# TravisWheelerLab/BATH

Hardware: AMD Instinct MI355X
Metric: DP Gcells/s + residues/s through bathsearch pipeline at 1/2/4/8 MI355X (higher is better)
Workload: dtype u8/i16 integer scores (SSV: exact binary16), f32 Forward

## Files before the change

bath_amd/__init__.py:

```python
import ctypes as C
import os
import subprocess

import numpy as np

_HERE = os.path.dirname(os.path.abspath(__file__))
_ROOT = os.path.dirname(_HERE)
LIB_PATH = os.environ.get("BATH_HIP_LIBRARY") or os.path.join(_HERE, "libbathhip.so")

OK, EINVAL, ERANGE, ENORESULT = 0, 11, 16, 19
KP, K, NEVPARAM = 29, 20, 8
LOGSUM_TABLE, LOGSUM_EXACT, LOGSUM_TABLE_SERIAL, LOGSUM_CONTEXT = 0, 1, 2, 3
LOGSUM_ODDS = 4
ENSEMBLE_SERIAL, ENSEMBLE_STREAMS_HOST, ENSEMBLE_STREAMS_DEVICE = 0, 1, 2
ENSEMBLE_MODES = {"serial": ENSEMBLE_SERIAL, "streams": ENSEMBLE_STREAMS_HOST, "device": ENSEMBLE_STREAMS_DEVICE}
ENS_SAMPLES = 200
ARITH_STRICT, ARITH_ODDS3, ARITH_ODDS = 0, 1, 2
ARITH_MODES = {"strict": ARITH_STRICT, "odds3": ARITH_ODDS3, "odds": ARITH_ODDS}
ENS_OK, ENS_IMPOSSIBLE, ENS_STEP_CAP, ENS_SEG_OVERFLOW = 0, 1, 2, 3
ENS_REGION_OK, ENS_REGION_NO_TRACES = 0, 1

DNA_SYMS = "ACGT-RYMKSWHBVDN*~"
AMINO_SYMS = "ACDEFGHIKLMNPQRSTVWY-BJZOUX*~"

# ... 150 lines not shown
    "bath_hmmfile_count": (C.c_int, [C.c_char_p]),
    "bath_hmmfile_read": (C.c_int, [C.c_char_p, C.c_int, C.POINTER(C.POINTER(_Hmm))]),
    "bath_hmm_destroy": (None, [C.POINTER(_Hmm)]),
    "bath_gencode_basic": (C.c_int, [C.c_int, _u8p]),
    "bath_profile_config": (C.c_int, [C.POINTER(_Hmm), C.c_int, C.POINTER(C.POINTER(_Profile))]),
    "bath_profile_destroy": (None, [C.POINTER(_Profile)]),
    "bath_fs_profile_config": (C.c_int, [C.POINTER(_Hmm), _u8p, C.c_int, C.c_int, C.POINTER(C.POINTER(_FsProfile))]),
    "bath_fs_profile_destroy": (None, [C.POINTER(_FsProfile)]),
    "bath_hip_init": (C.c_int, [C.c_int, C.POINTER(_vp)]),
    "bath_hip_finalize": (None, [_vp]),
    "bath_hip_last_error": (C.c_char_p, [_vp]),
    "bath_hip_synchronize": (C.c_int, [_vp]),
    "bath_hip_stream": (_vp, [_vp]),
    "bath_hip_set_fs_strict": (C.c_int, [_vp, C.c_int]),
    "bath_hip_set_fwd_group": (C.c_int, [_vp, C.c_int]),
    "bath_hip_set_fs_serial": (C.c_int, [_vp, C.c_int]),
    "bath_hip_set_fs_odds": (C.c_int, [_vp, C.c_int]),
    "bath_hip_set_fs5_odds": (C.c_int, [_vp, C.c_int]),
    "bath_hip_set_fs_ensemble": (C.c_int, [_vp, C.c_int]),
    "bath_hip_fs_ensemble_counters": (C.c_int, [_vp, _i64p, _i64p, _i64p]),
    "bath_hip_set_std_ensemble": (C.c_int, [_vp, C.c_int]),
    "bath_hip_std_ensemble_counters": (C.c_int, [_vp, _i64p, _i64p, _i64p]),
    "bath_hip_std_region_ensembles": (C.c_int, [_vp, _vp, _vp, _i32p, C.c_uint32, _i32p, _i32p, _i32p, C.c_int64, _i64p, _i32p, _f32p, C.c_int64, _i64p]),
    "bath_selftest_std_ensemble": (C.c_int, [C.c_int, C.c_int, _f32p, _f32p, C.c_float, C.c_float, C.c_float, _u8p, C.c_int, _f32p, _f32p, C.c_uint32, _i32p, _i32p,
                                             _i32p, C.c_int, _i32p, _f32p, _i32p, C.c_int, _i32p]),
    "bath_selftest_std_ens_walk": (C.c_int, [C.c_int, _f32p, C.c_float, C.c_float, C.c_float, C.c_int, _f32p, _f32p, C.c_uint32, _i32p, _i32p, C.c_int, _i32p]),
    "bath_hip_fs5_region_ensembles": (C.c_int, [_vp, _vp, _vp, C.c_uint32, _i32p, _i32p, _i32p, C.c_int64, _i64p, _i32p, C.c_int64, _i64p]),
    "bath_selftest_fs_ensemble_seeded": (C.c_int, [C.c_int, _f32p, C.c_float, C.c_float, C.c_float, C.c_int, C.c_int, _f32p, _f32p, C.c_uint32, _i32p, C.c_int, _i32p]),
    "bath_selftest_fs_ensemble_streams": (C.c_int, [C.c_int, _f32p, C.c_float, C.c_float, C.c_float, C.c_int, C.c_int, _f32p, _f32p, C.c_uint32,
                                                    _i32p, _i32p, _i32p, C.c_int, _i32p, _i32p, C.c_int, _i32p]),
# ... 297 lines not shown
        if st != OK:
            raise BathError("%s failed (%d): %s" % (what, st, lib().bath_hip_last_error(self._h).decode()))

    def synchronize(self):
        self._check(lib().bath_hip_synchronize(self._h), "synchronize")

    def trim(self):
        self._check(lib().bath_hip_trim(self._h), "trim")

    def set_fs_strict(self, on=True):
        self._check(lib().bath_hip_set_fs_strict(self._h, 1 if on else 0), "set_fs_strict")

    def set_fwd_group(self, mode):
        self._check(lib().bath_hip_set_fwd_group(self._h, int(mode)), "set_fwd_group")

    def set_fs_odds(self, on=True):
        self._check(lib().bath_hip_set_fs_odds(self._h, 1 if on else 0), "set_fs_odds")

    def set_fs5_odds(self, on=True):
        self._check(lib().bath_hip_set_fs5_odds(self._h, 1 if on else 0), "set_fs5_odds")

    def set_fs_ensemble(self, mode):
        self._check(lib().bath_hip_set_fs_ensemble(self._h, ENSEMBLE_MODES.get(mode, mode)), "set_fs_ensemble")

    def fs_ensemble_counters(self):
        a, b, c = C.c_int64(0), C.c_int64(0), C.c_int64(0)
        self._check(lib().bath_hip_fs_ensemble_counters(self._h, C.byref(a), C.byref(b), C.byref(c)), "fs_ensemble_counters")
        return {"bound_fallbacks": a.value, "overflow_fallbacks": b.value, "matrix_bytes_kept": c.value}

    def set_std_ensemble(self, mode):
# ... 1279 lines not shown
```

bath_amd/csrc/bath_common.hpp:

```cpp
#pragma once
#include <set>
#include <atomic>
#include <hip/hip_runtime.h>

#include <cstdint>
#include <chrono>
#include <cstdio>
#include <cstdlib>
#include <cstring>
#include <condition_variable>
#include <functional>
#include <mutex>
#include <string>
#include <thread>
#include <vector>

#include "bath_hip.h"
#include "bath_tilings.hpp"
#include "bath_slots.hpp"

namespace bath {

inline hipError_t allow_max_lds(const void *fn) {
  static std::mutex mu;
// ... 116 lines not shown

}

struct bath_hip_ctx;
namespace bath {
extern std::atomic<int> g_ctx_total, g_ctx_internal;
inline int host_contexts() { return g_ctx_total.load() - g_ctx_internal.load(); }
inline void mark_internal(bath_hip_ctx *c);
}
struct bath_hip_ctx {
  int device = 0;
  hipStream_t stream = nullptr;
  hipStream_t tail_stream = nullptr;
  hipStream_t side_stream = nullptr;
  hipEvent_t ev_fork = nullptr, ev_join = nullptr;
  hipStream_t copy_stream = nullptr;
  hipDeviceProp_t prop{};
  int fs_strict = 1;
  int fs_odds = 0;
  int fs5_odds = 0;
  int fwd_group = 0;
  int fs_ensemble = 0;
  std::atomic<int64_t> fs_ens_bound_fallbacks{0}, fs_ens_overflow_fallbacks{0}, fs_ens_bytes_kept{0};
  int std_ensemble = 0;
  std::atomic<int64_t> std_ens_serial_fallbacks{0}, std_ens_twin_fallbacks{0}, std_ens_kernel_regions{0};
  int fs_serial = -1;
  uint64_t tabs_uid = 0;
  const void *tabs_ptr = nullptr;
  uint64_t fsw_pad_uid = 0;
  int orf_tables_id = -1;
  std::string err;
  void set_error(const std::string &m) { err = m; }
  std::vector<float> fsw_len_terms;
  bath::SlotArray<bath::Scratch, bath::DevBuf> scratch;
  bath::SlotArray<bath::Pinned, bath::HostBuf> stage;
  template <class T> int stage_upload(bath::Pinned slot, void *dst, const T *src, size_t n, hipStream_t s) {
// ... 187 lines not shown
```

bath_amd/csrc/bath_pipeline.hip:

```cpp
#include <algorithm>
#include <cmath>
#include <cstring>
#include <cstdlib>
#include <map>
#include <thread>

#include "bath_common.hpp"
#include "bath_kernels.hpp"
#include "bath_launch.hpp"
#include "host_model.hpp"

using namespace bath;

namespace bath {

static const double kLog2 = 0.69314718055994529;

enum { FLAG_VIT_RUN = 1, FLAG_HAS_WIN = 2 };

struct Counters {
  int cand_count, todo_msv, todo_vit, todo_ssvb, todo_vit2, todo_fwd, win_count, overflow;
  int todo_lb;
  int fwd_next;
  unsigned long long n_orfs, orf_res;
  unsigned long long n_past_msv, n_past_bias, n_past_vit, n_past_fwd;
  unsigned long long pos_past_msv, pos_past_bias, pos_past_vit, pos_past_fwd;
  unsigned long long res_vit, res_fwd;
  unsigned long long res_seen;
};

struct Params {
  double F1, F2, F3, F4;
  int do_bias, fs_pipe, minlen;
  float evparam[BATH_NEVPARAM];
};

template <int NR, int G>
// ... 378 lines not shown
  for (int dx = 0; dx < 6; dx++) {
    float n0 = 0.f, n1 = 0.f, den = 0.f;
    if (dx == 5) { for (int y = 0; y < 20; y++) { n0 += bgf[y]; n1 += compo[y]; den += bgf[y]; } }
    else {
      const int a = min(mem[dx][0], mem[dx][1]), b = max(mem[dx][0], mem[dx][1]);
      n0 += bgf[a]; n1 += compo[a]; den += bgf[a];
      if (b != a) { n0 += bgf[b]; n1 += compo[b]; den += bgf[b]; }
    }
    eo[2 * (21 + dx)] = den > 0.f ? n0 / den : 0.f;
    eo[2 * (21 + dx) + 1] = den > 0.f ? n1 / den : 0.f;
  }
}

enum { PV_TODO_LB = 0, PV_TODO_FWD = 1, PV_NL = 2 };
enum { PV_N_VIT = 0, PV_POS_VIT, PV_RES_FWD, PV_NS };
__global__ __launch_bounds__(256) void post_vit_kernel(Cand cand, int cand_cap, Counters *__restrict__ ctr, Params p, int32_t *__restrict__ todo_lb, int32_t *__restrict__ todo_fwd) {
  __shared__ BlockTally<PV_NL, PV_NS, 512> tally;
  tally_reset(tally);
  const TallyOut<PV_NL, PV_NS> out{{todo_lb, todo_fwd}, {&ctr->todo_lb, &ctr->todo_fwd}, {&ctr->n_past_vit, &ctr->pos_past_vit, &ctr->res_fwd}};
  const int ncand = min(ctr->cand_count, cand_cap);
  for (int c0 = blockIdx.x * blockDim.x; c0 < ncand; c0 += gridDim.x * blockDim.x) {
    if (tally_lists_full(tally)) tally_write_lists(tally, out);
    const int c = c0 + threadIdx.x;
    bool past = c < ncand && cand.stage[c] == 2;
    if (past && (cand.flags[c] & FLAG_VIT_RUN)) {
      const float seqsc = (float)((double)(cand.vfsc[c] - cand.filtersc[c]) / kLog2);
      const double P = d_gumbel_surv(seqsc, p.evparam[2], p.evparam[3]);
      cand.P[c] = P;
      if (P > p.F2) { cand.kminmax[2 * c] = 1 << 30; cand.kminmax[2 * c + 1] = 0; past = false; }
    }
    if (!past) continue;
    const int L = cand.len[c];
    tally_add(tally, PV_N_VIT, 1ull); tally_add(tally, PV_POS_VIT, (unsigned long long)L * 3ull);
    if (p.do_bias && cand.kminmax[2 * c] <= cand.kminmax[2 * c + 1]) {
      cand.flags[c] |= FLAG_HAS_WIN;
      tally_push(tally, PV_TODO_LB, c);
      continue;
    }
    cand.stage[c] = 3;
    tally_push(tally, PV_TODO_FWD, c); tally_add(tally, PV_RES_FWD, (unsigned long long)L);
  }
  tally_finish(tally, out);
}

__host__ __device__ __forceinline__ float compo_term(float bg, int base_b, int sc, float scale_b) {
  const float lo = ((float)base_b - (float)sc) / scale_b;
  return bg * expf(lo);
}
__global__ void compo_terms_kernel(const float *__restrict__ bgf, int base_b, float scale_b, float *__restrict__ terms ) {
  const int x = blockIdx.x, sc = threadIdx.x;
  terms[x * 256 + sc] = compo_term(bgf[x], base_b, sc, scale_b);
}

__global__ __launch_bounds__(64) void local_compo_kernel(Cand cand, const Counters *__restrict__ ctr, int M, const uint8_t *__restrict__ ssv_scores,
                                                         const float *__restrict__ terms, const int32_t *__restrict__ todo_lb, float *__restrict__ compo_out ) {
  const int lane = threadIdx.x, g = lane / 20, x = lane % 20;
  const int ntodo = ctr->todo_lb;
  for (int base = blockIdx.x * 3; base < ntodo; base += gridDim.x * 3) {
    const int job = base + g;
    if (g >= 3 || job >= ntodo) continue;
    const int c = todo_lb[job];
    int k_start = cand.kminmax[2 * c], k_end = cand.kminmax[2 * c + 1];
    const int k_len = k_end - k_start + 1;
    if (k_len < 20) { k_start -= (20 - k_len) / 2; k_end += (20 - k_len) / 2; }
    k_start = max(1, k_start); k_end = min(M, k_end);
    const float *tx = terms + x * 256;
    float acc = 0.0f;
    for (int k = k_start; k <= k_end; k++) acc += tx[ssv_scores[(size_t)k * kKp + x]];
    compo_out[(size_t)job * 20 + x] = acc;
  }
}

__global__ __launch_bounds__(64) void post_vit_local_kernel(Cand cand, Counters *__restrict__ ctr, Params p, const uint8_t *__restrict__ pool, int M,
                                                            const float *__restrict__ bgf, const float *__restrict__ compo_in,
                                                            const float *__restrict__ p1_tab, const float *__restrict__ lt1_tab, const float *__restrict__ lt2_tab,
                                                            const int32_t *__restrict__ todo_lb, int32_t *__restrict__ todo_vit2, int32_t *__restrict__ todo_fwd) {
  __shared__ float s_eo[64][kKp * 2 + 1];
  __shared__ BlockTally<2, 2, 128> tally;
  tally_reset(tally);
  const TallyOut<2, 2> out{{todo_vit2, todo_fwd}, {&ctr->todo_vit2, &ctr->todo_fwd}, {&ctr->res_vit, &ctr->res_fwd}};
  const int ntodo = ctr->todo_lb;
  for (int job0 = blockIdx.x * blockDim.x; job0 < ntodo; job0 += gridDim.x * blockDim.x) {
    if (tally_lists_full(tally)) tally_write_lists(tally, out);
    const int job = job0 + threadIdx.x;
    if (job >= ntodo) continue;
    const int c = todo_lb[job];
    const int L = cand.len[c];
    const float usc = cand.usc[c];
    float filtersc = cand.filtersc[c];
    const float vfsc = (cand.flags[c] & FLAG_VIT_RUN) ? cand.vfsc[c] : -INFINITY;
    float compo[20];
    for (int y = 0; y < 20; y++) compo[y] = compo_in[(size_t)job * 20 + y];
    float *eo = s_eo[threadIdx.x];
    local_compo_finish(compo, bgf, eo);
    float lf = bias_forward(pool + cand.off[c], L, M, eo, p1_tab[L]);
    lf = (lf + lt1_tab[L]) + lt2_tab[L];
// ... 115 lines not shown
  float *d_bgf = om->d_compo_terms + 20 * 256;
  BATH_HIP_TRY(ctx, hipMemcpyAsync(d_bgf, kAminoBg, 20 * sizeof(float), hipMemcpyHostToDevice, ctx->stream));
  hipLaunchKernelGGL(compo_terms_kernel, dim3(20), dim3(256), 0, ctx->stream, d_bgf, (int)om->base_b, om->scale_b, om->d_compo_terms);
  BATH_HIP_TRY(ctx, hipGetLastError());
  BATH_HIP_TRY(ctx, hipStreamSynchronize(ctx->stream));
  return BATH_OK;
}

static int wave_grid_blocks(bath_hip_ctx *ctx) { return ctx->prop.multiProcessorCount * 8; }

struct PipelineWork {
  Cand cand;
  int cand_cap = 0;
  uint8_t *pool = nullptr;
  int32_t *todo_msv = nullptr, *todo_vit = nullptr, *todo_ssvb = nullptr, *todo_vit2 = nullptr, *todo_fwd = nullptr, *todo_sorted = nullptr;
  int *len_bins = nullptr;
  WindowRec *wins = nullptr;
  int win_cap = 0;
  Counters *ctr = nullptr;
};

template <class T>
static T *carve(char *&p, size_t n) {
  T *r = reinterpret_cast<T *>(p);
  p += (n * sizeof(T) + 255) / 256 * 256;
  return r;
}

static size_t layout(PipelineWork &w, char *base, int cap, int win_cap) {
  char *p = base;
// ... 1 lines not shown
  w.cand_cap = cap; w.win_cap = std::max(2 * cap, win_cap);
  if (win_cap == 0) {
    static const int forced = [] { const char *e = std::getenv("BATH_HIP_TEST_WINCAP"); return e ? std::atoi(e) : 0; }();
    if (forced > 0) w.win_cap = forced;
  }
  w.ctr = carve<Counters>(p, 1);
  w.cand.window = carve<int64_t>(p, n); w.cand.off = carve<int64_t>(p, n); w.cand.P = carve<double>(p, n);
  w.cand.sf = carve<int32_t>(p, n); w.cand.startj = carve<int32_t>(p, n); w.cand.len = carve<int32_t>(p, n);
  w.cand.msv_status = carve<int32_t>(p, n); w.cand.vit_status = carve<int32_t>(p, n); w.cand.fwd_status = carve<int32_t>(p, n); w.cand.stage = carve<int32_t>(p, n);
  w.cand.flags = carve<int32_t>(p, n); w.cand.kminmax = carve<int32_t>(p, 2 * n);
  w.cand.usc = carve<float>(p, n); w.cand.nullsc = carve<float>(p, n); w.cand.filtersc = carve<float>(p, n);
  w.cand.vfsc = carve<float>(p, n); w.cand.fwdsc = carve<float>(p, n);
  w.cand.v = carve<int16_t>(p, n);
  w.todo_msv = carve<int32_t>(p, n); w.todo_vit = carve<int32_t>(p, n); w.todo_ssvb = carve<int32_t>(p, n);
  w.todo_vit2 = carve<int32_t>(p, n); w.todo_fwd = carve<int32_t>(p, n); w.todo_sorted = carve<int32_t>(p, n);
  w.len_bins = carve<int>(p, 2048);
  w.wins = carve<WindowRec>(p, (size_t)w.win_cap);
  return (size_t)(p - base);
}

}

extern "C" int bath_selftest_compo_terms(int base_b, float scale_b, float *terms) {
  if (!terms || !(scale_b > 0.f)) return BATH_EINVAL;
  for (int x = 0; x < 20; x++)
    for (int sc = 0; sc < 256; sc++) terms[x * 256 + sc] = bath::compo_term(kAminoBg[x], base_b, sc, scale_b);
  return BATH_OK;
}

extern "C" void bath_pipeline_params_default(bath_pipeline_params *p, int fs_pipe) {
// ... 190 lines not shown
      BATH_HIP_TRY(ctx, hipEventRecord(ev[e++], ctx->stream));
    } else {
      hipLaunchKernelGGL(classify_kernel, dim3(dec_blocks), dim3(256), 0, ctx->stream, W.cand, W.cand_cap, W.ctr, om->lt.d_tjb, mc, W.todo_msv);
      BATH_HIP_TRY(ctx, hipGetLastError());
      if ((st = launch_msv_wave(ctx, om, cv, W.todo_msv, cap, W.cand.usc, W.cand.msv_status, &W.ctr->todo_msv, !few_msv)) != BATH_OK) return st;
      BATH_HIP_TRY(ctx, hipEventRecord(ev[e++], ctx->stream));
      hipLaunchKernelGGL(f1_bias_kernel, dim3(dec_blocks), dim3(256), 0, ctx->stream, W.cand, W.cand_cap, W.ctr, P, W.pool, M, f1t, W.todo_vit, W.todo_ssvb);
      BATH_HIP_TRY(ctx, hipGetLastError());
      BATH_HIP_TRY(ctx, hipEventRecord(ev[e++], ctx->stream));
    }
    wa.d_filtersc = W.cand.filtersc; wa.d_ssv_scores = d_ssvsc; wa.d_wins = W.wins; wa.d_win_count = &W.ctr->win_count; wa.win_cap = W.win_cap;
    wa.d_kminmax = W.cand.kminmax;
    auto launch_ssvb = [&](hipStream_t stream) -> int {
      return launch_ssv_bath(ctx, stream, om, W.cand, W.ctr, W.todo_ssvb, W.pool, d_ssvsc, mc, invP_f1, W.wins, W.win_cap);
    };
    bool ssvb_done = false;
    if (vit_lane_supported(om) && !few_cands) {
      if ((st = launch_vit_sorted(ctx, om, cv, W.todo_vit, cap, &W.ctr->todo_vit, W.cand.len, W.len_bins, W.todo_sorted, W.cand.vfsc, W.cand.vit_status, &wa,
                                  launch_ssvb)) != BATH_OK) return st;
      ssvb_done = true;
    } else if ((st = launch_vit_wave(ctx, om, cv, W.todo_vit, cap, W.cand.vfsc, W.cand.vit_status, &wa, &W.ctr->todo_vit)) != BATH_OK) return st;
    BATH_HIP_TRY(ctx, hipEventRecord(ev[e++], ctx->stream));
    if (!ssvb_done && (st = launch_ssvb(ctx->stream)) != BATH_OK) return st;
    BATH_HIP_TRY(ctx, hipGetLastError());
    BATH_HIP_TRY(ctx, hipEventRecord(ev[e++], ctx->stream));
    hipLaunchKernelGGL(post_vit_kernel, dim3(dec_blocks), dim3(256), 0, ctx->stream, W.cand, W.cand_cap, W.ctr, P, W.todo_msv , W.todo_fwd);
    if (P.do_bias) {
      DevBuf &b_compo = ctx->scratch[Scratch::kLocalCompoSums];
      BATH_HIP_TRY(ctx, b_compo.reserve((size_t)W.cand_cap * 20 * 4 + 256));
      float *d_compo = b_compo.as<float>();
      hipLaunchKernelGGL(local_compo_kernel, dim3(16384), dim3(64), 0, ctx->stream, W.cand, W.ctr, M, d_ssvsc, om->d_compo_terms, W.todo_msv, d_compo);
      hipLaunchKernelGGL(post_vit_local_kernel, dim3(std::max(1, dec_blocks)), dim3(64), 0, ctx->stream, W.cand, W.ctr, P, W.pool, M, d_bgf, d_compo,
                         om->lt.d_p1, om->lt.d_lt1, om->lt.d_lt2, W.todo_msv, W.todo_vit2, W.todo_fwd);
    }
    BATH_HIP_TRY(ctx, hipGetLastError());
    if ((st = launch_vit_wave(ctx, om, cv, W.todo_vit2, cap, W.cand.vfsc, W.cand.vit_status, nullptr, &W.ctr->todo_vit2)) != BATH_OK) return st;
    hipLaunchKernelGGL(post_vit2_kernel, dim3(64), dim3(256), 0, ctx->stream, W.cand, W.ctr, P, W.todo_vit2, W.todo_fwd);
    BATH_HIP_TRY(ctx, hipGetLastError());
    BATH_HIP_TRY(ctx, hipEventRecord(ev[e++], ctx->stream));
    ctx->fwd_rows_kept = nullptr; ctx->fwd_rows_off = nullptr;
    float *d_keep = nullptr; int64_t *d_keep_off = nullptr;
    if (ctx->keep_fwd_rows) {
      constexpr int64_t kKeepFloats = (int64_t)8 << 20;
      DevBuf &b_rows = ctx->scratch[Scratch::kCascadeFwdRows], &b_roff = ctx->scratch[Scratch::kCascadeFwdRowOffsets];
      BATH_HIP_TRY(ctx, b_rows.reserve((size_t)kKeepFloats * sizeof(float) + 64)); BATH_HIP_TRY(ctx, b_roff.reserve((size_t)cap * sizeof(int64_t) + 64));
      d_keep = b_rows.as<float>(); d_keep_off = b_roff.as<int64_t>();
      hipLaunchKernelGGL(fwd_keep_offsets_kernel, dim3(1), dim3(64), 0, ctx->stream, W.todo_fwd, &W.ctr->todo_fwd, W.cand.len, d_keep_off, kKeepFloats);
      BATH_HIP_TRY(ctx, hipGetLastError());
    }
    const bool fwd_group = !d_keep && fwd_group_supported(om) && ctx->fwd_group != 2;
    if (fwd_group) {
      if ((st = launch_len_sort(ctx, W.todo_fwd, &W.ctr->todo_fwd, W.cand.len, W.len_bins, W.todo_sorted)) != BATH_OK) return st;
// ... 2 lines not shown
    const int64_t fwd_launches = (d_keep ? 1 : 0) + (fwd_group ? 4 : 1) + 1;
    if (d_keep) { ctx->fwd_rows_kept = d_keep; ctx->fwd_rows_off = d_keep_off; }
    hipLaunchKernelGGL(final_kernel, dim3(dec_blocks), dim3(256), 0, ctx->stream, W.cand, W.ctr, P, W.todo_fwd);
    BATH_HIP_TRY(ctx, hipGetLastError());
    BATH_HIP_TRY(ctx, hipEventRecord(ev[e++], ctx->stream));

    BATH_HIP_TRY(ctx, hipMemcpyAsync(&hc, W.ctr, sizeof(Counters), hipMemcpyDeviceToHost, ctx->stream));
    BATH_HIP_TRY(ctx, hipStreamSynchronize(ctx->stream));
    if (hc.overflow || hc.cand_count > cap || hc.win_count > W.win_cap) {
      if (attempt >= 4) { ctx->set_error("candidate / window buffers overflowed repeatedly"); return BATH_EMEM; }
      if (hc.overflow || hc.cand_count > cap) cap = std::max<int64_t>(cap * 2, (int64_t)hc.cand_count + 1024);
      if (hc.win_count > W.win_cap) win_need = hc.win_count + hc.win_count / 4 + 1024;
      continue;
    }
    static const char *names[] = {"translate_orfs", "ssv_f1", "classify_msv", "f1_bias", "viterbi_windows", "ssv_windows", "post_vit", "forward_final"};
    const int64_t launches[] = {4, 1, msv_stage ? 1 : 2, msv_stage ? 0 : 1, 4, 1, 3, fwd_launches};
    ctx->timings.clear();
    for (int i = 0; i + 1 < e; i++) {
      float ms = 0.f;
      BATH_HIP_TRY(ctx, hipEventElapsedTime(&ms, ev[i], ev[i + 1]));
      ctx->timings.push_back(StageTiming{names[i], ms, launches[i]});
    }
    break;
  }

  if (stats) {
    stats->nres = nres; stats->n_orfs = (int64_t)hc.n_orfs;
    stats->n_past_msv = (int64_t)hc.n_past_msv; stats->n_past_bias = (int64_t)hc.n_past_bias;
    stats->n_past_vit = (int64_t)hc.n_past_vit; stats->n_past_fwd = (int64_t)hc.n_past_fwd;
    stats->pos_past_msv = (int64_t)hc.pos_past_msv; stats->pos_past_bias = (int64_t)hc.pos_past_bias;
    stats->pos_past_vit = (int64_t)hc.pos_past_vit; stats->pos_past_fwd = (int64_t)hc.pos_past_fwd;
// ... 87 lines not shown
    mark_internal(lane);
    const char *pe = std::getenv("BATH_HIP_LANE_PRIO");
    if (!(pe && pe[0] == '0')) {
      int lo = 0, hi = 0;
      if (hipDeviceGetStreamPriorityRange(&lo, &hi) == hipSuccess && lo != hi) {
        (void)hipStreamDestroy(lane->stream);
        const char *te = std::getenv("BATH_HIP_TAIL_PRIO");
        const bool tails = te && te[0] == '1';
        const int prio = tails ? (ctx->lanes.empty() ? std::min(lo, hi + 1) : lo) : (ctx->lanes.empty() ? hi : lo);
        if (hipStreamCreateWithPriority(&lane->stream, hipStreamNonBlocking, prio) != hipSuccess) { ctx->set_error("hipStreamCreateWithPriority"); return BATH_EFAIL; }
        if (tails && hipStreamCreateWithPriority(&lane->tail_stream, hipStreamNonBlocking, hi) != hipSuccess) { ctx->set_error("hipStreamCreateWithPriority"); return BATH_EFAIL; }
      }
    }
    ctx->lanes.push_back(lane);
  }
  for (bath_hip_ctx *lane : ctx->lanes) { lane->fs_strict = ctx->fs_strict; lane->fs_odds = ctx->fs_odds; lane->fs5_odds = ctx->fs5_odds; lane->fwd_group = ctx->fwd_group; }
  if ((st = ensure_parts(ctx, dna, K)) != BATH_OK) return st;
  std::vector<bath_pipeline_stats> pst((size_t)K);
  std::vector<const bath_orf_result *> pres((size_t)K, nullptr);
  std::vector<int64_t> pn((size_t)K, 0);
  std::vector<int> rc((size_t)K, BATH_OK);
  states->assign((size_t)K, FilterState{});
  if (!ctx->ev_lanes) BATH_HIP_TRY(ctx, hipEventCreateWithFlags(&ctx->ev_lanes, hipEventDisableTiming));
  BATH_HIP_TRY(ctx, hipEventRecord(ctx->ev_lanes, ctx->stream));
  for (int k = 0; k < K; k++) BATH_HIP_TRY(ctx, hipStreamWaitEvent(ctx->lanes[(size_t)k]->stream, ctx->ev_lanes, 0));
  if (!ctx->lane_pool) ctx->lane_pool = new LanePool();
  ctx->lane_pool->run(K, [&](int k) {
    bath_hip_ctx *lane = ctx->lanes[(size_t)k];
    rc[(size_t)k] = run_filters(lane, om, dna->parts[(size_t)k], prm, &pst[(size_t)k], results ? &pres[(size_t)k] : nullptr, &pn[(size_t)k], &(*states)[(size_t)k]);
    if (rc[(size_t)k] == BATH_OK) rc[(size_t)k] = after(k, lane, dna->parts[(size_t)k], (*states)[(size_t)k]);
  });
// ... 511 lines not shown
```

bath_amd/csrc/bath_profile.hip:

```cpp
#include <atomic>
#include <cctype>
#include <cmath>
#include <cstring>

#include "bath_common.hpp"
#include "host_model.hpp"

using namespace bath;

namespace bath {

static const double kLog2 = 0.69314718055994529;

double gumbel_surv(double x, double mu, double lambda) {
  double ey = -std::exp(-lambda * (x - mu));
  if (std::fabs(ey) < 5e-9) return -ey;
  return 1.0 - std::exp(ey);
}
double gumbel_invsurv(double p, double mu, double lambda) {
  double lp = (p < 5e-9) ? (std::pow(p, p) - 1) / p : std::log(-1. * std::log(1 - p));
  return mu - lp / lambda;
}
double exp_surv(double x, double mu, double lambda) { return (x < mu) ? 1.0 : std::exp(-lambda * (x - mu)); }

// ... 67 lines not shown

}

int bath_hip_oprofile::ensure_len_tables(int maxL) const { return bath::build_len_tables(this, maxL); }


namespace bath { std::atomic<int> g_ctx_total{0}, g_ctx_internal{0}; }

extern "C" int bath_hip_init(int device, bath_hip_ctx **out) {
  *out = nullptr;
  int ndev = 0;
  if (hipGetDeviceCount(&ndev) != hipSuccess || ndev <= 0) return BATH_ENODEVICE;
  if (device < 0 || device >= ndev) return BATH_EINVAL;
  bath_hip_ctx *ctx = new bath_hip_ctx();
  ctx->device = device;
  if (const char *e = std::getenv("BATH_HIP_SYNC")) {
    static const bool once = [&] {
      (void)hipSetDevice(device);
      const unsigned fl = (e[0] == 'b') ? hipDeviceScheduleBlockingSync : (e[0] == 'y') ? hipDeviceScheduleYield : hipDeviceScheduleSpin;
      if (hipSetDeviceFlags(fl) != hipSuccess) (void)hipGetLastError();
      return true;
    }();
    (void)once;
  }
  if (hipSetDevice(device) != hipSuccess || hipGetDeviceProperties(&ctx->prop, device) != hipSuccess ||
      hipStreamCreateWithFlags(&ctx->stream, hipStreamNonBlocking) != hipSuccess) {
    delete ctx;
    return BATH_ENODEVICE;
  }
  bath::g_ctx_total.fetch_add(1);
// ... 13 lines not shown
  if (ctx->ev_lanes) (void)hipEventDestroy(ctx->ev_lanes);
  if (ctx->tail_stream) (void)hipStreamDestroy(ctx->tail_stream);
  if (ctx->aux) { bath_hip_finalize(ctx->aux); ctx->aux = nullptr; }
  if (ctx->aux2) { bath_hip_finalize(ctx->aux2); ctx->aux2 = nullptr; }
  if (ctx->aux3) { bath_hip_finalize(ctx->aux3); ctx->aux3 = nullptr; }
  for (auto &b : ctx->scratch) b.release();
  for (auto &b : ctx->pinned) b.release();
  for (auto &b : ctx->stage) b.release();
  ctx->results_pinned.release();
  for (auto e : ctx->ev_pool) (void)hipEventDestroy(e);
  for (auto e : ctx->span_events) (void)hipEventDestroy(e);
  if (ctx->ev_fork) (void)hipEventDestroy(ctx->ev_fork);
  if (ctx->ev_join) (void)hipEventDestroy(ctx->ev_join);
  if (ctx->copy_stream) (void)hipStreamDestroy(ctx->copy_stream);
  if (ctx->side_stream) (void)hipStreamDestroy(ctx->side_stream);
  (void)hipStreamDestroy(ctx->stream);
  delete ctx;
}

extern "C" int bath_hip_trim(bath_hip_ctx *ctx) {
  if (!ctx) return BATH_EINVAL;
  BATH_HIP_TRY(ctx, hipSetDevice(ctx->device));
  BATH_HIP_TRY(ctx, hipStreamSynchronize(ctx->stream));
  delete ctx->lane_pool; ctx->lane_pool = nullptr;
  for (bath_hip_ctx *lane : ctx->lanes) bath_hip_finalize(lane);
  ctx->lanes.clear();
  if (ctx->aux) { bath_hip_finalize(ctx->aux); ctx->aux = nullptr; }
  if (ctx->aux2) { bath_hip_finalize(ctx->aux2); ctx->aux2 = nullptr; }
  if (ctx->aux3) { bath_hip_finalize(ctx->aux3); ctx->aux3 = nullptr; }
  if (ctx->tail_stream) { (void)hipStreamDestroy(ctx->tail_stream); ctx->tail_stream = nullptr; }
  if (ctx->copy_stream) { (void)hipStreamSynchronize(ctx->copy_stream); (void)hipStreamDestroy(ctx->copy_stream); ctx->copy_stream = nullptr; }
  if (ctx->side_stream) {
    (void)hipStreamSynchronize(ctx->side_stream); (void)hipStreamDestroy(ctx->side_stream); ctx->side_stream = nullptr;
    if (ctx->ev_fork) { (void)hipEventDestroy(ctx->ev_fork); ctx->ev_fork = nullptr; }
    if (ctx->ev_join) { (void)hipEventDestroy(ctx->ev_join); ctx->ev_join = nullptr; }
  }
  ctx->fs_std_orfs.clear(); ctx->fs_std_pool = nullptr; ctx->fs_keep_xoff.clear(); ctx->fs_regions_all.clear();
  ctx->d_records = nullptr; ctx->n_records = 0;
  return BATH_OK;
}

extern "C" const char *bath_hip_last_error(const bath_hip_ctx *ctx) { return ctx ? ctx->err.c_str() : "no context"; }

extern "C" int bath_hip_synchronize(bath_hip_ctx *ctx) {
  BATH_HIP_TRY(ctx, hipSetDevice(ctx->device));
  BATH_HIP_TRY(ctx, hipStreamSynchronize(ctx->stream));
  return BATH_OK;
}

extern "C" void *bath_hip_stream(bath_hip_ctx *ctx) { return (void *)ctx->stream; }
extern "C" int bath_hip_kernel_times(bath_hip_ctx *ctx, int max, bath_kernel_time *out) {
// ... 19 lines not shown
}

extern "C" int bath_hip_set_fs_strict(bath_hip_ctx *ctx, int on) {
  if (!ctx) return BATH_EINVAL;
  ctx->fs_strict = on ? 1 : 0;
  if (!on && ctx->aux3) { bath_hip_finalize(ctx->aux3); ctx->aux3 = nullptr; }
  for (bath_hip_ctx *l : ctx->lanes) l->fs_strict = ctx->fs_strict;
  return BATH_OK;
}

extern "C" int bath_hip_set_fwd_group(bath_hip_ctx *ctx, int mode) {
  if (!ctx) return BATH_EINVAL;
  if (mode < 0 || mode > 2) { ctx->set_error("bath_hip_set_fwd_group: mode must be 0, 1 or 2"); return BATH_EINVAL; }
  ctx->fwd_group = mode;
  for (bath_hip_ctx *l : ctx->lanes) l->fwd_group = mode;
  return BATH_OK;
}

extern "C" int bath_hip_set_fs_odds(bath_hip_ctx *ctx, int on) {
  if (!ctx) return BATH_EINVAL;
  ctx->fs_odds = on ? 1 : 0;
  for (bath_hip_ctx *l : ctx->lanes) l->fs_odds = ctx->fs_odds;
  return BATH_OK;
}

extern "C" int bath_hip_set_fs5_odds(bath_hip_ctx *ctx, int on) {
  if (!ctx) return BATH_EINVAL;
  ctx->fs5_odds = on ? 1 : 0;
  for (bath_hip_ctx *l : ctx->lanes) l->fs5_odds = ctx->fs5_odds;
  return BATH_OK;
// ... 471 lines not shown
```

bath_amd/csrc/bath_viterbi.hip:

```cpp
#include <algorithm>
#include <cstdlib>
#include <functional>

#include "bath_common.hpp"
#include "bath_kernels.hpp"
#include "bath_launch.hpp"

using namespace bath;

namespace bath {

__device__ __forceinline__ s16x2 pk_adds(s16x2 a, s16x2 b) { return __builtin_elementwise_add_sat(a, b); }
__device__ __forceinline__ s16x2 pk_max(s16x2 a, s16x2 b) { return __builtin_elementwise_max(a, b); }
__device__ __forceinline__ s16x2 as_s2(unsigned v) { return __builtin_bit_cast(s16x2, v); }
__device__ __forceinline__ unsigned as_u(s16x2 v) { return __builtin_bit_cast(unsigned, v); }

struct VitLaneTables {
  const int16_t *rw;
  int rw_pitch_bytes;
  const uint32_t *tw2;
  const int16_t *rank;
};

struct VitLaneConsts {
// ... 6 lines not shown

typedef uint32_t u32x16 __attribute__((ext_vector_type(16)));

template <int NR>
#ifndef BATH_VIT_WAVES
#define BATH_VIT_WAVES 1
#endif
__global__ __launch_bounds__(256, (NR <= 76 ? BATH_VIT_WAVES : 1)) void vit_lane_kernel(SeqView sq, VitLaneTables tb, const uint32_t *__restrict__ tw2g, VitLaneConsts c, const int16_t *__restrict__ xwmove_tab,
                                                          const uint8_t *__restrict__ tjb_tab, const int32_t *__restrict__ todo, int64_t ntodo,
                                                          const int *__restrict__ ntodo_dev, const int *__restrict__ skip_dev, float *__restrict__ sc, int32_t *__restrict__ status,
                                                          const float *__restrict__ filtersc, const uint8_t *__restrict__ ssv_scores,
                                                          WindowRec *__restrict__ wins, int *__restrict__ win_count, int win_cap, int32_t *__restrict__ kminmax) {
  extern __shared__ __attribute__((aligned(16))) char lds[];
  char *s_rw = lds;
  int16_t *s_rank = reinterpret_cast<int16_t *>(lds + 30 * tb.rw_pitch_bytes);
  {
    const uint32_t *src = reinterpret_cast<const uint32_t *>(tb.rw);
    uint32_t *dst = reinterpret_cast<uint32_t *>(s_rw);
    for (int i = threadIdx.x; i < 30 * tb.rw_pitch_bytes / 4; i += blockDim.x) dst[i] = src[i];
    for (int i = threadIdx.x; i < 2 * NR; i += blockDim.x) s_rank[i] = tb.rank[i];
  }
  __syncthreads();
  if (ntodo_dev) ntodo = *ntodo_dev;
  const int64_t t = (int64_t)blockIdx.x * blockDim.x + threadIdx.x + (skip_dev ? *skip_dev : 0);
  if (t - (threadIdx.x & 63) >= ntodo) return;
  const bool live = t < ntodo;
  const int64_t sid = live ? (todo ? (int64_t)todo[t] : t) : (todo ? (int64_t)todo[0] : 0);
  const int L = live ? sq.len[sid] : 0;
  const uint8_t *s = sq.data + sq.off[sid];
  const int Lw = wave_max_i32(L);
// ... 279 lines not shown
```

include/bath_hip.h:

```cpp
#ifndef BATH_HIP_H
#define BATH_HIP_H

#include <stdint.h>
#include <stddef.h>

#ifdef __cplusplus
extern "C" {
#endif

#define BATH_OK          0
#define BATH_EFAIL       1
#define BATH_EMEM        5
#define BATH_EFORMAT     7
#define BATH_EINVAL     11
#define BATH_ERANGE     16
#define BATH_ENORESULT  19
#define BATH_ENODEVICE  40

#define BATH_KP_AMINO   29
#define BATH_K_AMINO    20
#define BATH_KP_DNA     18
#define BATH_NEVPARAM    8
#define BATH_FTAU        4
#define BATH_FLAMBDA     5
// ... 49 lines not shown
int  bath_profile_config(const bath_hmm *hmm, int L, bath_profile **ret);
void bath_profile_destroy(bath_profile *gm);
int  bath_fs_profile_config(const bath_hmm *hmm, const uint8_t basic[64], int codon_lengths, int L_amino,
                            bath_fs_profile **ret);
void bath_fs_profile_destroy(bath_fs_profile *gm);

int         bath_hip_init(int device, bath_hip_ctx **ctx);
void        bath_hip_finalize(bath_hip_ctx *ctx);
const char *bath_hip_last_error(const bath_hip_ctx *ctx);
int         bath_hip_synchronize(bath_hip_ctx *ctx);
int         bath_hip_trim(bath_hip_ctx *ctx);
void       *bath_hip_stream(bath_hip_ctx *ctx);
int         bath_hip_set_fs_strict(bath_hip_ctx *ctx, int on);
int         bath_hip_set_fs_odds(bath_hip_ctx *ctx, int on);
int         bath_hip_set_fwd_group(bath_hip_ctx *ctx, int mode);
int         bath_hip_set_fs5_odds(bath_hip_ctx *ctx, int on);
#define BATH_ENSEMBLE_SERIAL 0
#define BATH_ENSEMBLE_STREAMS_HOST 1
#define BATH_ENSEMBLE_STREAMS_DEVICE 2
int         bath_hip_set_fs_ensemble(bath_hip_ctx *ctx, int mode);
int         bath_hip_fs_ensemble_counters(bath_hip_ctx *ctx, int64_t *bound_fallbacks, int64_t *overflow_fallbacks, int64_t *matrix_bytes_kept);
int         bath_hip_set_std_ensemble(bath_hip_ctx *ctx, int mode);
int         bath_hip_std_ensemble_counters(bath_hip_ctx *ctx, int64_t *serial_fallbacks, int64_t *twin_fallbacks, int64_t *kernel_regions);
int         bath_hip_set_fs_serial(bath_hip_ctx *ctx, int on);

int  bath_hip_oprofile_convert(bath_hip_ctx *ctx, const bath_profile *gm, bath_hip_oprofile **ret);
void bath_hip_oprofile_destroy(bath_hip_oprofile *om);
int  bath_hip_oprofile_set_consensus(bath_hip_oprofile *om, const char *consensus);
int  bath_hip_oprofile_M(const bath_hip_oprofile *om);

// ... 401 lines not shown
```

Baseline: 215.2 billion.

## Overlap SSV-bath strong branch with Viterbi post-processing on a side stream

Splits the post-Viterbi tail into two branches: candidates that skipped Viterbi (strong SSV) go through SSV-bath, post-vit, bias and the Viterbi rerun on a new non-blocking stream. The Viterbi-run candidates are post-processed concurrently on the main stream, with fork and join events around the pair. Separate lb todo lists and compo buffers keep the two branches from sharing state. The Viterbi kernel also gains an early exit for blocks past the work count, so idle blocks skip the LDS table load. The change adds stream and event overhead and two branches appending to shared todo_fwd/todo_vit2 counters through atomics, which may change list order.

```diff
diff --git a/bath_amd/__init__.py b/bath_amd/__init__.py
--- a/bath_amd/__init__.py
+++ b/bath_amd/__init__.py
@@ -188,6 +188,7 @@
     "bath_hip_stream": (_vp, [_vp]),
     "bath_hip_set_fs_strict": (C.c_int, [_vp, C.c_int]),
     "bath_hip_set_fwd_group": (C.c_int, [_vp, C.c_int]),
+    "bath_hip_set_tail_branches": (C.c_int, [_vp, C.c_int]),
     "bath_hip_set_fs_serial": (C.c_int, [_vp, C.c_int]),
     "bath_hip_set_fs_odds": (C.c_int, [_vp, C.c_int]),
     "bath_hip_set_fs5_odds": (C.c_int, [_vp, C.c_int]),
@@ -515,6 +516,9 @@
     def set_fwd_group(self, mode):
         self._check(lib().bath_hip_set_fwd_group(self._h, int(mode)), "set_fwd_group")
 
+    def set_tail_branches(self, mode):
+        self._check(lib().bath_hip_set_tail_branches(self._h, int(mode)), "set_tail_branches")
+
     def set_fs_odds(self, on=True):
         self._check(lib().bath_hip_set_fs_odds(self._h, 1 if on else 0), "set_fs_odds")
 
diff --git a/bath_amd/csrc/bath_common.hpp b/bath_amd/csrc/bath_common.hpp
--- a/bath_amd/csrc/bath_common.hpp
+++ b/bath_amd/csrc/bath_common.hpp
@@ -154,12 +154,15 @@
   hipStream_t tail_stream = nullptr;
   hipStream_t side_stream = nullptr;
   hipEvent_t ev_fork = nullptr, ev_join = nullptr;
+  hipStream_t strong_stream = nullptr;
+  hipEvent_t ev_strong_fork = nullptr, ev_strong_join = nullptr;
   hipStream_t copy_stream = nullptr;
   hipDeviceProp_t prop{};
   int fs_strict = 1;
   int fs_odds = 0;
   int fs5_odds = 0;
   int fwd_group = 0;
+  int tail_branches = 0;
   int fs_ensemble = 0;
   std::atomic<int64_t> fs_ens_bound_fallbacks{0}, fs_ens_overflow_fallbacks{0}, fs_ens_bytes_kept{0};
   int std_ensemble = 0;
diff --git a/bath_amd/csrc/bath_pipeline.hip b/bath_amd/csrc/bath_pipeline.hip
--- a/bath_amd/csrc/bath_pipeline.hip
+++ b/bath_amd/csrc/bath_pipeline.hip
@@ -21,6 +21,7 @@
 struct Counters {
   int cand_count, todo_msv, todo_vit, todo_ssvb, todo_vit2, todo_fwd, win_count, overflow;
   int todo_lb;
+  int todo_lb_strong;
   int fwd_next;
   unsigned long long n_orfs, orf_res;
   unsigned long long n_past_msv, n_past_bias, n_past_vit, n_past_fwd;
@@ -429,16 +430,20 @@
 
 enum { PV_TODO_LB = 0, PV_TODO_FWD = 1, PV_NL = 2 };
 enum { PV_N_VIT = 0, PV_POS_VIT, PV_RES_FWD, PV_NS };
-__global__ __launch_bounds__(256) void post_vit_kernel(Cand cand, int cand_cap, Counters *__restrict__ ctr, Params p, int32_t *__restrict__ todo_lb, int32_t *__restrict__ todo_fwd) {
+enum { PV_ALL = 0, PV_VITERBI = 1, PV_STRONG = 2 };
+__global__ __launch_bounds__(256) void post_vit_kernel(Cand cand, int cand_cap, Counters *__restrict__ ctr, Params p, int which, int32_t *__restrict__ todo_lb,
+                                                       int *__restrict__ n_lb, int32_t *__restrict__ todo_fwd) {
   __shared__ BlockTally<PV_NL, PV_NS, 512> tally;
   tally_reset(tally);
-  const TallyOut<PV_NL, PV_NS> out{{todo_lb, todo_fwd}, {&ctr->todo_lb, &ctr->todo_fwd}, {&ctr->n_past_vit, &ctr->pos_past_vit, &ctr->res_fwd}};
+  const TallyOut<PV_NL, PV_NS> out{{todo_lb, todo_fwd}, {n_lb, &ctr->todo_fwd}, {&ctr->n_past_vit, &ctr->pos_past_vit, &ctr->res_fwd}};
   const int ncand = min(ctr->cand_count, cand_cap);
   for (int c0 = blockIdx.x * blockDim.x; c0 < ncand; c0 += gridDim.x * blockDim.x) {
     if (tally_lists_full(tally)) tally_write_lists(tally, out);
     const int c = c0 + threadIdx.x;
     bool past = c < ncand && cand.stage[c] == 2;
-    if (past && (cand.flags[c] & FLAG_VIT_RUN)) {
+    const bool vit_run = past && (cand.flags[c] & FLAG_VIT_RUN);
+    if (which != PV_ALL && vit_run != (which == PV_VITERBI)) past = false;
+    if (past && vit_run) {
       const float seqsc = (float)((double)(cand.vfsc[c] - cand.filtersc[c]) / kLog2);
       const double P = d_gumbel_surv(seqsc, p.evparam[2], p.evparam[3]);
       cand.P[c] = P;
@@ -468,9 +473,10 @@
 }
 
 __global__ __launch_bounds__(64) void local_compo_kernel(Cand cand, const Counters *__restrict__ ctr, int M, const uint8_t *__restrict__ ssv_scores,
-                                                         const float *__restrict__ terms, const int32_t *__restrict__ todo_lb, float *__restrict__ compo_out ) {
+                                                         const float *__restrict__ terms, const int32_t *__restrict__ todo_lb, const int *__restrict__ n_lb,
+                                                         float *__restrict__ compo_out ) {
   const int lane = threadIdx.x, g = lane / 20, x = lane % 20;
-  const int ntodo = ctr->todo_lb;
+  const int ntodo = *n_lb;
   for (int base = blockIdx.x * 3; base < ntodo; base += gridDim.x * 3) {
     const int job = base + g;
     if (g >= 3 || job >= ntodo) continue;
@@ -489,12 +495,13 @@
 __global__ __launch_bounds__(64) void post_vit_local_kernel(Cand cand, Counters *__restrict__ ctr, Params p, const uint8_t *__restrict__ pool, int M,
                                                             const float *__restrict__ bgf, const float *__restrict__ compo_in,
                                                             const float *__restrict__ p1_tab, const float *__restrict__ lt1_tab, const float *__restrict__ lt2_tab,
-                                                            const int32_t *__restrict__ todo_lb, int32_t *__restrict__ todo_vit2, int32_t *__restrict__ todo_fwd) {
+                                                            const int32_t *__restrict__ todo_lb, const int *__restrict__ n_lb, int32_t *__restrict__ todo_vit2,
+                                                            int32_t *__restrict__ todo_fwd) {
   __shared__ float s_eo[64][kKp * 2 + 1];
   __shared__ BlockTally<2, 2, 128> tally;
   tally_reset(tally);
   const TallyOut<2, 2> out{{todo_vit2, todo_fwd}, {&ctr->todo_vit2, &ctr->todo_fwd}, {&ctr->res_vit, &ctr->res_fwd}};
-  const int ntodo = ctr->todo_lb;
+  const int ntodo = *n_lb;
   for (int job0 = blockIdx.x * blockDim.x; job0 < ntodo; job0 += gridDim.x * blockDim.x) {
     if (tally_lists_full(tally)) tally_write_lists(tally, out);
     const int job = job0 + threadIdx.x;
@@ -640,6 +647,7 @@
   int cand_cap = 0;
   uint8_t *pool = nullptr;
   int32_t *todo_msv = nullptr, *todo_vit = nullptr, *todo_ssvb = nullptr, *todo_vit2 = nullptr, *todo_fwd = nullptr, *todo_sorted = nullptr;
+  int32_t *todo_lb_strong = nullptr;
   int *len_bins = nullptr;
   WindowRec *wins = nullptr;
   int win_cap = 0;
@@ -671,6 +679,7 @@
   w.cand.v = carve<int16_t>(p, n);
   w.todo_msv = carve<int32_t>(p, n); w.todo_vit = carve<int32_t>(p, n); w.todo_ssvb = carve<int32_t>(p, n);
   w.todo_vit2 = carve<int32_t>(p, n); w.todo_fwd = carve<int32_t>(p, n); w.todo_sorted = carve<int32_t>(p, n);
+  w.todo_lb_strong = carve<int32_t>(p, n);
   w.len_bins = carve<int>(p, 2048);
   w.wins = carve<WindowRec>(p, (size_t)w.win_cap);
   return (size_t)(p - base);
@@ -891,28 +900,77 @@
     auto launch_ssvb = [&](hipStream_t stream) -> int {
       return launch_ssv_bath(ctx, stream, om, W.cand, W.ctr, W.todo_ssvb, W.pool, d_ssvsc, mc, invP_f1, W.wins, W.win_cap);
     };
-    bool ssvb_done = false;
-    if (vit_lane_supported(om) && !few_cands) {
-      if ((st = launch_vit_sorted(ctx, om, cv, W.todo_vit, cap, &W.ctr->todo_vit, W.cand.len, W.len_bins, W.todo_sorted, W.cand.vfsc, W.cand.vit_status, &wa,
-                                  launch_ssvb)) != BATH_OK) return st;
-      ssvb_done = true;
-    } else if ((st = launch_vit_wave(ctx, om, cv, W.todo_vit, cap, W.cand.vfsc, W.cand.vit_status, &wa, &W.ctr->todo_vit)) != BATH_OK) return st;
-    BATH_HIP_TRY(ctx, hipEventRecord(ev[e++], ctx->stream));
-    if (!ssvb_done && (st = launch_ssvb(ctx->stream)) != BATH_OK) return st;
-    BATH_HIP_TRY(ctx, hipGetLastError());
-    BATH_HIP_TRY(ctx, hipEventRecord(ev[e++], ctx->stream));
-    hipLaunchKernelGGL(post_vit_kernel, dim3(dec_blocks), dim3(256), 0, ctx->stream, W.cand, W.cand_cap, W.ctr, P, W.todo_msv , W.todo_fwd);
+    float *d_compo = nullptr;
     if (P.do_bias) {
       DevBuf &b_compo = ctx->scratch[Scratch::kLocalCompoSums];
-      BATH_HIP_TRY(ctx, b_compo.reserve((size_t)W.cand_cap * 20 * 4 + 256));
-      float *d_compo = b_compo.as<float>();
-      hipLaunchKernelGGL(local_compo_kernel, dim3(16384), dim3(64), 0, ctx->stream, W.cand, W.ctr, M, d_ssvsc, om->d_compo_terms, W.todo_msv, d_compo);
-      hipLaunchKernelGGL(post_vit_local_kernel, dim3(std::max(1, dec_blocks)), dim3(64), 0, ctx->stream, W.cand, W.ctr, P, W.pool, M, d_bgf, d_compo,
-                         om->lt.d_p1, om->lt.d_lt1, om->lt.d_lt2, W.todo_msv, W.todo_vit2, W.todo_fwd);
-    }
-    BATH_HIP_TRY(ctx, hipGetLastError());
-    if ((st = launch_vit_wave(ctx, om, cv, W.todo_vit2, cap, W.cand.vfsc, W.cand.vit_status, nullptr, &W.ctr->todo_vit2)) != BATH_OK) return st;
-    hipLaunchKernelGGL(post_vit2_kernel, dim3(64), dim3(256), 0, ctx->stream, W.cand, W.ctr, P, W.todo_vit2, W.todo_fwd);
+      BATH_HIP_TRY(ctx, b_compo.reserve((size_t)W.cand_cap * 2 * 20 * 4 + 256));
+      d_compo = b_compo.as<float>();
+    }
+    int64_t post_launches = 0;
+    auto post_vit_chain = [&](int which) {
+      const bool strong = which == PV_STRONG;
+      int32_t *todo_lb = strong ? W.todo_lb_strong : W.todo_msv ;
+      int *n_lb = strong ? &W.ctr->todo_lb_strong : &W.ctr->todo_lb;
+      float *compo = d_compo ? d_compo + (strong ? (size_t)W.cand_cap * 20 : 0) : nullptr;
+      hipLaunchKernelGGL(post_vit_kernel, dim3(dec_blocks), dim3(256), 0, ctx->stream, W.cand, W.cand_cap, W.ctr, P, which, todo_lb, n_lb, W.todo_fwd);
+      post_launches++;
+      if (P.do_bias) {
+        hipLaunchKernelGGL(local_compo_kernel, dim3(16384), dim3(64), 0, ctx->stream, W.cand, W.ctr, M, d_ssvsc, om->d_compo_terms, todo_lb, n_lb, compo);
+        hipLaunchKernelGGL(post_vit_local_kernel, dim3(std::max(1, dec_blocks)), dim3(64), 0, ctx->stream, W.cand, W.ctr, P, W.pool, M, d_bgf, compo,
+                           om->lt.d_p1, om->lt.d_lt1, om->lt.d_lt2, todo_lb, n_lb, W.todo_vit2, W.todo_fwd);
+        post_launches += 2;
+      }
+    };
+    auto vit_rerun = [&]() -> int {
+      const int rc = launch_vit_wave(ctx, om, cv, W.todo_vit2, cap, W.cand.vfsc, W.cand.vit_status, nullptr, &W.ctr->todo_vit2);
+      if (rc != BATH_OK) return rc;
+      hipLaunchKernelGGL(post_vit2_kernel, dim3(64), dim3(256), 0, ctx->stream, W.cand, W.ctr, P, W.todo_vit2, W.todo_fwd);
+      post_launches += 2;
+      return BATH_OK;
+    };
+    const bool vit_lane = vit_lane_supported(om) && !few_cands;
+    int64_t vit_launches = vit_lane ? 5 : 1, ssvb_launches = 0;
+    if (ctx->tail_branches != 2 && vit_lane) {
+      if (!ctx->strong_stream) {
+        BATH_HIP_TRY(ctx, hipStreamCreateWithFlags(&ctx->strong_stream, hipStreamNonBlocking));
+        BATH_HIP_TRY(ctx, hipEventCreateWithFlags(&ctx->ev_strong_fork, hipEventDisableTiming));
+        BATH_HIP_TRY(ctx, hipEventCreateWithFlags(&ctx->ev_strong_join, hipEventDisableTiming));
+      }
+      BATH_HIP_TRY(ctx, hipEventRecord(ctx->ev_strong_fork, ctx->stream));
+      BATH_HIP_TRY(ctx, hipStreamWaitEvent(ctx->strong_stream, ctx->ev_strong_fork, 0));
+      if ((st = launch_vit_sorted(ctx, om, cv, W.todo_vit, cap, &W.ctr->todo_vit, W.cand.len, W.len_bins, W.todo_sorted, W.cand.vfsc, W.cand.vit_status, &wa,
+                                  nullptr)) != BATH_OK) return st;
+      {
+        hipStream_t main_stream = ctx->stream;
+        ctx->stream = ctx->strong_stream;
+        st = launch_ssvb(ctx->stream);
+        post_launches++;
+        if (st == BATH_OK) { post_vit_chain(PV_STRONG); st = vit_rerun(); }
+        ctx->stream = main_stream;
+        if (st != BATH_OK) return st;
+      }
+      BATH_HIP_TRY(ctx, hipGetLastError());
+      BATH_HIP_TRY(ctx, hipEventRecord(ctx->ev_strong_join, ctx->strong_stream));
+      BATH_HIP_TRY(ctx, hipEventRecord(ev[e++], ctx->stream));
+      BATH_HIP_TRY(ctx, hipEventRecord(ev[e++], ctx->stream));
+      post_vit_chain(PV_VITERBI);
+      BATH_HIP_TRY(ctx, hipGetLastError());
+      BATH_HIP_TRY(ctx, hipStreamWaitEvent(ctx->stream, ctx->ev_strong_join, 0));
+    } else {
+      bool ssvb_done = false;
+      if (vit_lane) {
+        if ((st = launch_vit_sorted(ctx, om, cv, W.todo_vit, cap, &W.ctr->todo_vit, W.cand.len, W.len_bins, W.todo_sorted, W.cand.vfsc, W.cand.vit_status, &wa,
+                                    launch_ssvb)) != BATH_OK) return st;
+        ssvb_done = true; vit_launches++;
+      } else if ((st = launch_vit_wave(ctx, om, cv, W.todo_vit, cap, W.cand.vfsc, W.cand.vit_status, &wa, &W.ctr->todo_vit)) != BATH_OK) return st;
+      BATH_HIP_TRY(ctx, hipEventRecord(ev[e++], ctx->stream));
+      if (!ssvb_done) { if ((st = launch_ssvb(ctx->stream)) != BATH_OK) return st; ssvb_launches++; }
+      BATH_HIP_TRY(ctx, hipGetLastError());
+      BATH_HIP_TRY(ctx, hipEventRecord(ev[e++], ctx->stream));
+      post_vit_chain(PV_ALL);
+      BATH_HIP_TRY(ctx, hipGetLastError());
+      if ((st = vit_rerun()) != BATH_OK) return st;
+    }
     BATH_HIP_TRY(ctx, hipGetLastError());
     BATH_HIP_TRY(ctx, hipEventRecord(ev[e++], ctx->stream));
     ctx->fwd_rows_kept = nullptr; ctx->fwd_rows_off = nullptr;
@@ -945,7 +1003,7 @@
       continue;
     }
     static const char *names[] = {"translate_orfs", "ssv_f1", "classify_msv", "f1_bias", "viterbi_windows", "ssv_windows", "post_vit", "forward_final"};
-    const int64_t launches[] = {4, 1, msv_stage ? 1 : 2, msv_stage ? 0 : 1, 4, 1, 3, fwd_launches};
+    const int64_t launches[] = {4, 1, msv_stage ? 1 : 2, msv_stage ? 0 : 1, vit_launches, ssvb_launches, post_launches, fwd_launches};
     ctx->timings.clear();
     for (int i = 0; i + 1 < e; i++) {
       float ms = 0.f;
@@ -1063,7 +1121,7 @@
     }
     ctx->lanes.push_back(lane);
   }
-  for (bath_hip_ctx *lane : ctx->lanes) { lane->fs_strict = ctx->fs_strict; lane->fs_odds = ctx->fs_odds; lane->fs5_odds = ctx->fs5_odds; lane->fwd_group = ctx->fwd_group; }
+  for (bath_hip_ctx *lane : ctx->lanes) { lane->fs_strict = ctx->fs_strict; lane->fs_odds = ctx->fs_odds; lane->fs5_odds = ctx->fs5_odds; lane->fwd_group = ctx->fwd_group; lane->tail_branches = ctx->tail_branches; }
   if ((st = ensure_parts(ctx, dna, K)) != BATH_OK) return st;
   std::vector<bath_pipeline_stats> pst((size_t)K);
   std::vector<const bath_orf_result *> pres((size_t)K, nullptr);
diff --git a/bath_amd/csrc/bath_profile.hip b/bath_amd/csrc/bath_profile.hip
--- a/bath_amd/csrc/bath_profile.hip
+++ b/bath_amd/csrc/bath_profile.hip
@@ -105,6 +105,7 @@
   if (device < 0 || device >= ndev) return BATH_EINVAL;
   bath_hip_ctx *ctx = new bath_hip_ctx();
   ctx->device = device;
+  if (const char *e = std::getenv("BATH_HIP_TAIL_BRANCHES")) { const int m = std::atoi(e); if (m >= 0 && m <= 2) ctx->tail_branches = m; }
   if (const char *e = std::getenv("BATH_HIP_SYNC")) {
     static const bool once = [&] {
       (void)hipSetDevice(device);
@@ -148,6 +149,9 @@
   if (ctx->ev_join) (void)hipEventDestroy(ctx->ev_join);
   if (ctx->copy_stream) (void)hipStreamDestroy(ctx->copy_stream);
   if (ctx->side_stream) (void)hipStreamDestroy(ctx->side_stream);
+  if (ctx->ev_strong_fork) (void)hipEventDestroy(ctx->ev_strong_fork);
+  if (ctx->ev_strong_join) (void)hipEventDestroy(ctx->ev_strong_join);
+  if (ctx->strong_stream) (void)hipStreamDestroy(ctx->strong_stream);
   (void)hipStreamDestroy(ctx->stream);
   delete ctx;
 }
@@ -169,6 +173,11 @@
     if (ctx->ev_fork) { (void)hipEventDestroy(ctx->ev_fork); ctx->ev_fork = nullptr; }
     if (ctx->ev_join) { (void)hipEventDestroy(ctx->ev_join); ctx->ev_join = nullptr; }
   }
+  if (ctx->strong_stream) {
+    (void)hipStreamSynchronize(ctx->strong_stream); (void)hipStreamDestroy(ctx->strong_stream); ctx->strong_stream = nullptr;
+    if (ctx->ev_strong_fork) { (void)hipEventDestroy(ctx->ev_strong_fork); ctx->ev_strong_fork = nullptr; }
+    if (ctx->ev_strong_join) { (void)hipEventDestroy(ctx->ev_strong_join); ctx->ev_strong_join = nullptr; }
+  }
   ctx->fs_std_orfs.clear(); ctx->fs_std_pool = nullptr; ctx->fs_keep_xoff.clear(); ctx->fs_regions_all.clear();
   ctx->d_records = nullptr; ctx->n_records = 0;
   return BATH_OK;
@@ -218,6 +227,14 @@
   if (mode < 0 || mode > 2) { ctx->set_error("bath_hip_set_fwd_group: mode must be 0, 1 or 2"); return BATH_EINVAL; }
   ctx->fwd_group = mode;
   for (bath_hip_ctx *l : ctx->lanes) l->fwd_group = mode;
+  return BATH_OK;
+}
+
+extern "C" int bath_hip_set_tail_branches(bath_hip_ctx *ctx, int mode) {
+  if (!ctx) return BATH_EINVAL;
+  if (mode < 0 || mode > 2) { ctx->set_error("bath_hip_set_tail_branches: mode must be 0, 1 or 2"); return BATH_EINVAL; }
+  ctx->tail_branches = mode;
+  for (bath_hip_ctx *l : ctx->lanes) l->tail_branches = mode;
   return BATH_OK;
 }
 
diff --git a/bath_amd/csrc/bath_viterbi.hip b/bath_amd/csrc/bath_viterbi.hip
--- a/bath_amd/csrc/bath_viterbi.hip
+++ b/bath_amd/csrc/bath_viterbi.hip
@@ -44,6 +44,7 @@
   extern __shared__ __attribute__((aligned(16))) char lds[];
   char *s_rw = lds;
   int16_t *s_rank = reinterpret_cast<int16_t *>(lds + 30 * tb.rw_pitch_bytes);
+  if ((int64_t)blockIdx.x * blockDim.x + (skip_dev ? *skip_dev : 0) >= (ntodo_dev ? (int64_t)*ntodo_dev : ntodo)) return;
   {
     const uint32_t *src = reinterpret_cast<const uint32_t *>(tb.rw);
     uint32_t *dst = reinterpret_cast<uint32_t *>(s_rw);
diff --git a/include/bath_hip.h b/include/bath_hip.h
--- a/include/bath_hip.h
+++ b/include/bath_hip.h
@@ -87,6 +87,7 @@
 int         bath_hip_set_fs_strict(bath_hip_ctx *ctx, int on);
 int         bath_hip_set_fs_odds(bath_hip_ctx *ctx, int on);
 int         bath_hip_set_fwd_group(bath_hip_ctx *ctx, int mode);
+int         bath_hip_set_tail_branches(bath_hip_ctx *ctx, int mode);
 int         bath_hip_set_fs5_odds(bath_hip_ctx *ctx, int on);
 #define BATH_ENSEMBLE_SERIAL 0
 #define BATH_ENSEMBLE_STREAMS_HOST 1
```

Result: no change. 215.4 billion, median of 2 (+0.1%).
